# yuanming-hu/exposure

Hardware: AMD Instinct MI355X
Metric: Mpixels/s through 8-step filter chain fwd+bwd (higher is better)
Workload: dtype f16; 1 GPU; 8-step filter chain (E,G,W,S+,T,Ct,BW,C) fwd+bwd, 64x512x512x3 f16 NHWC per GPU, one HIP kernel per filter step and direction; batch_per_gpu=64, global_batch=64, height=512, width=512, parallelism=image-sharded replicas x1 (no data-path collective), weak scaling, launch=hipGraph replay, 10 steps (330 captured launches) per replay, chain_streams=2, transport=none (one process)

## Files before the change

### exposure_amd/csrc/exposure_hip.hip

```cpp
#include <dlfcn.h>
#include <hip/hip_runtime.h>
#include <stdint.h>
#include <stdio.h>
#include <stdlib.h>
#include <string.h>
#include <mutex>
#include <vector>
#include <string>
#include <type_traits>

#include "../../include/exposure_hip.h"
#include "filter_math.h"
#include "pixel_io.h"
#include "kernel_common.h"
#include "host_common.h"

#ifndef EXPO_BWD_MIN_WAVES
#define EXPO_BWD_MIN_WAVES
#endif
#ifndef EXPO_CURVE_BWD_PREFETCH
#define EXPO_CURVE_BWD_PREFETCH 1
#endif
constexpr bool kFwdPrefetch = false;
constexpr bool kBwdPrefetch = true;
constexpr int kAccParts = 4;


namespace expo {

template <class F, typename T, bool VEC, bool PEN, class IO = IoCached>
__device__ __forceinline__ void fwd_body(const T* __restrict__ xi, T* __restrict__ yi,
                                         const float* __restrict__ prm, float* __restrict__ rec,
                                         int hw, int groups) {
  constexpr int PPL = PixTraits<T>::PPL;
  typename F::Prm q;
  if constexpr (!VEC) q = F::load(prm);
  float pen = 0.f;
  const int stride = gridDim.x * kThreads;
  constexpr bool kCurveTab = VEC && F::kLutFloats > 0;
  constexpr int kNC = kCurveTab ? F::NP / kCurveSteps : 1;
  __shared__ float2_lut ftab[kCurveTab ? kWaves : 1][32];
  float2_lut* const tab = ftab[kCurveTab ? (threadIdx.x >> 6) : 0];
  auto compute = [&](float* v, int g) {
    if constexpr (kCurveTab) {
      curve_lut_apply<kNC, PPL>(v, tab);
      if constexpr (PEN) {
#pragma unroll
        for (int j = 0; j < PPL * 3; ++j) {
          const float o = fmaxf(v[j] - 1.0f, 0.0f);
          pen = fmaf(o, o, pen);
        }
      }
      return;
    }
#pragma unroll
    for (int k = 0; k < PPL; ++k) {
      float y[3];
      F::fwd(q, v + 3 * k, y);
#pragma unroll
      for (int c = 0; c < 3; ++c) {
        v[3 * k + c] = y[c];
        if constexpr (PEN) {
          const float o = fmaxf(y[c] - 1.0f, 0.0f);
          pen = fmaf(o, o, pen);
        }
      }
    }
  };
  if constexpr (VEC) {
    const T* const ins[1] = {xi};
    stream_groups<T, 1, true, kFwdPrefetch, IO>(
        ins, yi, hw, blockIdx.x * kThreads + (threadIdx.x & ~63), stride,
        [&](float (&v)[1][PPL * 3], int g) { compute(v[0], g); },
        [&]() {
          q = F::load(prm);
          if constexpr (kCurveTab) curve_lut_build<kNC>(prm[(threadIdx.x & 63) % F::NP], tab);
        });
  } else {
    for (int g = blockIdx.x * kThreads + threadIdx.x; g < groups; g += stride) {
      float v[PPL * 3];
      load_slow<T>(xi, g, hw, v);
      compute(v, g);
      store_slow<T>(yi, g, hw, v);
    }
  }
  if constexpr (PEN) {
    float a[1] = {pen};
    block_reduce_record<1>(a, rec);
  }
}

template <class F, typename T, bool VEC, class IO>
__global__ __launch_bounds__(kThreads) void filter_fwd_kernel(const T* __restrict__ x, T* __restrict__ y,
                                                              const float* __restrict__ params,
                                                              int hw, int groups, int reverse) {
  const int n = reverse ? gridDim.y - 1 - blockIdx.y : blockIdx.y;
  const size_t off = size_t(n) * hw * 3;
  fwd_body<F, T, VEC, false, IO>(x + off, y + off, params + n * F::NP, nullptr, hw, groups);
}

template <class F, typename T, bool VEC, bool HAS_DX, bool PEN, int MODE, class IO = IoCached>
__device__ __forceinline__ void bwd_body(const T* __restrict__ xi, const T* __restrict__ dyi,
                                         T* __restrict__ dxi, const float* __restrict__ prm,
                                         float* __restrict__ rec, int hw, int groups, float pen_scale) {
  constexpr int PPL = PixTraits<T>::PPL;
  const typename F::Prm q = F::load(prm);
  __shared__ __attribute__((aligned(16))) float lut[F::kLutFloats > 0 ? F::kLutFloats : 4];
  constexpr bool kF16X = std::is_same<T, half_t>::value;
// ... 1700 lines not shown
  }
  if (cap != hipStreamCaptureStatusNone) return e;
  probe_helper(e);
  return e;
}
static ForkJoin* fork_join_for_device(hipStream_t caller = nullptr) {
  HelperEntry* e = helper_entry(caller, true);
  return e ? &e->fj : nullptr;
}
static std::mutex g_fork_join_mu;
static int chain_fork(ForkJoin* fj, hipStream_t s) {
  std::lock_guard<std::mutex> lock(g_fork_join_mu);
  HIP_TRY(hipEventRecord(fj->fork, s), "chain fork");
  HIP_TRY(hipStreamWaitEvent(fj->helper, fj->fork, 0), "chain fork");
  return EXPO_OK;
}
static int chain_join(ForkJoin* fj, hipStream_t s) {
  std::lock_guard<std::mutex> lock(g_fork_join_mu);
  HIP_TRY(hipEventRecord(fj->join, fj->helper), "chain join");
  HIP_TRY(hipStreamWaitEvent(s, fj->join, 0), "chain join");
  return EXPO_OK;
}
static bool chain_split(int n, int h, int w, int dtype) {
  static const int forced = getenv("EXPO_CHAIN_STREAMS") ? atoi(getenv("EXPO_CHAIN_STREAMS")) : 0;
  if (n < 2) return false;
  if (forced == 1) return false;
  if (forced >= 2) return true;
  const long bytes = long(n) * h * w * 3L * (dtype == EXPO_F16 ? 2L : 4L);
  return bytes >= (40L << 20) && bytes < (256L << 20);
}

static bool chain_snake(int n, int h, int w, int dtype) {
  static const int forced = getenv("EXPO_CHAIN_SNAKE") ? atoi(getenv("EXPO_CHAIN_SNAKE")) : -1;
  if (forced >= 0) return forced != 0;
  const long bytes = long(n) * h * w * 3L * (dtype == EXPO_F16 ? 2L : 4L);
  return bytes >= (256L << 20);
}

struct ChainChunk { int nb, np, lane; };
struct ChainPlan {
  std::vector<ChainChunk> chunks;
  bool two_lanes = false, snake = false;
};
static ChainPlan chain_plan(int n, int h, int w, int dtype) {
  static const int tile_mib = getenv("EXPO_CHAIN_TILE_MIB") ? atoi(getenv("EXPO_CHAIN_TILE_MIB")) : 96;
  ChainPlan plan;
  const long image_bytes = long(h) * w * 3L * (dtype == EXPO_F16 ? 2L : 4L);
  const long bytes = long(n) * image_bytes;
  int tiles = 1;
  static const long tile_min = long(getenv("EXPO_CHAIN_TILE_MIN_MIB") ? atoi(getenv("EXPO_CHAIN_TILE_MIN_MIB")) : 256) << 20;
  if (tile_mib > 0 && bytes >= tile_min && n > 1) {
    long tile_n = (long(tile_mib) << 20) / image_bytes;
    if (tile_n < 1) tile_n = 1;
    tiles = int((n + tile_n - 1) / tile_n);
  }
  if (tiles == 1) {
    plan.snake = chain_snake(n, h, w, dtype);
    plan.two_lanes = chain_split(n, h, w, dtype);
    const int n0 = plan.two_lanes ? n / 2 : n;
    plan.chunks.push_back({0, n0, 0});
    if (plan.two_lanes) plan.chunks.push_back({n0, n - n0, 1});
    return plan;
  }
  const int base = n / tiles, rem = n % tiles;
  plan.two_lanes = chain_split(base, h, w, dtype);
  int at = 0;
  for (int t = 0; t < tiles; ++t) {
    const int tn = base + (t < rem ? 1 : 0);
    const int n0 = (plan.two_lanes && tn >= 2) ? tn / 2 : tn;
    plan.chunks.push_back({at, n0, 0});
    if (n0 < tn) plan.chunks.push_back({at + n0, tn - n0, 1});
    at += tn;
  }
  return plan;
}

static int chain_fuse_steps(const ChainPlan& plan) {
  static const int forced = env_int("EXPO_CHAIN_FUSE_STEPS", 0);
  if (plan.snake) return 1;
  const int k = forced > 0 ? forced : kChainFuseMax;
  return k < kChainFuseMax ? k : kChainFuseMax;
}

extern "C" {

int expo_version(void) { return EXPO_ABI_VERSION; }

const char* expo_last_error(void) { return g_err.c_str(); }

#ifndef EXPO_SOURCE_DIGEST
#define EXPO_SOURCE_DIGEST "unknown"
#endif
const char* expo_build_info(void) { return EXPO_SOURCE_DIGEST; }

int expo_num_filter_params(int filter_id) {
  if (filter_id < 0 || filter_id >= EXPO_NUM_FILTERS) return -1;
  return kNumParams[filter_id];
}

size_t expo_workspace_bytes(int n, int h, int w, int dtype) {
  if (check_common(n, h, w, dtype) != EXPO_OK || n == 0) return 0;
  const int bx = geom_bx_max(n, h, w, dtype);
  return ws_step_bytes(n, bx);
}

int expo_filter_fwd(int filter_id, const void* x, void* y, const float* params, int n, int h, int w, int dtype,
                    void* stream) {
  if (int rc = check_common(n, h, w, dtype)) return rc;
  if (filter_id < 0 || filter_id >= EXPO_NUM_FILTERS) return fail(EXPO_E_BADARG, "filter_id out of range");
  if (n == 0) return EXPO_OK;
  if (!x || !y || !params) return fail(EXPO_E_BADARG, "null pointer");
  hipStream_t s = static_cast<hipStream_t>(stream);
  return dtype == EXPO_F16 ? fwd_by_id<half_t>(filter_id, x, y, params, n, h, w, s)
                           : fwd_by_id<float>(filter_id, x, y, params, n, h, w, s);
}

static int filter_bwd_common(int filter_id, const void* x, const void* dy, void* dx, const float* params,
                             float* dparams, int n, int h, int w, int dtype, int hsv_grad_mode, void* workspace,
                             size_t workspace_bytes, void* stream, bool accum) {
  if (int rc = check_common(n, h, w, dtype)) return rc;
  if (filter_id < 0 || filter_id >= EXPO_NUM_FILTERS) return fail(EXPO_E_BADARG, "filter_id out of range");
  if (hsv_grad_mode != 0 && hsv_grad_mode != 1) return fail(EXPO_E_BADARG, "hsv_grad_mode must be 0 or 1");
  if (n == 0) return EXPO_OK;
  if (!x || !dy || !params || !dparams) return fail(EXPO_E_BADARG, "null pointer");
  hipStream_t s = static_cast<hipStream_t>(stream);
  const int bx = geom_bx(bwd_geom_kind(filter_id), n, h, w, dtype);
  float* records;
  if (int rc = ws_check(workspace, workspace_bytes, n, bx, 1, &records)) return rc;
  const int rc = dtype == EXPO_F16
                     ? bwd_by_id<half_t>(filter_id, x, dy, dx, params, records, n, h, w, hsv_grad_mode, s)
                     : bwd_by_id<float>(filter_id, x, dy, dx, params, records, n, h, w, hsv_grad_mode, s);
  if (rc) return rc;
  FinishArgs fa{};
  fa.s[0] = FinishStep{params, dparams, nullptr, records, nullptr, kFinFilter, filter_id, accum ? 1 : 0, 0.f, bx};
  return launch_finish(fa, 1, n, s);
}

int expo_filter_bwd(int filter_id, const void* x, const void* dy, void* dx, const float* params, float* dparams,
                    int n, int h, int w, int dtype, int hsv_grad_mode, void* workspace, size_t workspace_bytes,
                    void* stream) {
  return filter_bwd_common(filter_id, x, dy, dx, params, dparams, n, h, w, dtype, hsv_grad_mode, workspace,
                           workspace_bytes, stream, false);
}

int expo_filter_bwd_accumulate(int filter_id, const void* x, const void* dy, void* dx, const float* params,
                               float* dparams, int n, int h, int w, int dtype, int hsv_grad_mode, void* workspace,
                               size_t workspace_bytes, void* stream) {
  return filter_bwd_common(filter_id, x, dy, dx, params, dparams, n, h, w, dtype, hsv_grad_mode, workspace,
                           workspace_bytes, stream, true);
}

int expo_filter_apply_fwd(int filter_id, const void* x, void* y, const float* params, const float* mask_params,
                          float maximum_sharpness, float minimum_strength, int n, int h, int w, int dtype,
                          void* stream) {
  if (int rc = check_common(n, h, w, dtype)) return rc;
  if (filter_id < 0 || filter_id >= EXPO_NUM_FILTERS) return fail(EXPO_E_BADARG, "filter_id out of range");
  if (n == 0) return EXPO_OK;
  if (!x || !y || !params || !mask_params) return fail(EXPO_E_BADARG, "null pointer");
  hipStream_t s = static_cast<hipStream_t>(stream);
  return dtype == EXPO_F16 ? apply_fwd_by_id<half_t>(filter_id, x, y, params, mask_params, maximum_sharpness,
                                                     minimum_strength, n, h, w, s)
                           : apply_fwd_by_id<float>(filter_id, x, y, params, mask_params, maximum_sharpness,
                                                    minimum_strength, n, h, w, s);
}

int expo_filter_apply_bwd(int filter_id, const void* x, const void* dy, void* dx, const float* params,
// ... 159 lines not shown
    int cnt = 1;
    for (int i = 0; i < steps && !rc; i += cnt) {
      cnt = steps - i < fuse ? steps - i : fuse;
      if (cnt > 1) {
        rc = chain_steps_fwd(filter_ids + i, cnt, acts + i, params + i, ck.nb, ck.np, h, w, dtype, n, sp);
      } else {
        const int rev = plan.snake ? (i & 1) : 0;
        const void* xin = static_cast<const char*>(acts[i]) + ioff;
        void* yout = static_cast<char*>(acts[i + 1]) + ioff;
        const float* prm = params[i] + size_t(ck.nb) * kNumParams[filter_ids[i]];
        rc = dtype == EXPO_F16 ? fwd_by_id<half_t>(filter_ids[i], xin, yout, prm, ck.np, h, w, sp, rev, n)
                               : fwd_by_id<float>(filter_ids[i], xin, yout, prm, ck.np, h, w, sp, rev, n);
      }
    }
  }
  if (fj) {
    const int jrc = chain_join(fj, s);
    if (!rc) rc = jrc;
  }
  return rc;
}

int expo_filter_bwd_records(int filter_id, const void* x, const void* dy, void* dx, const float* params, int n,
                            int h, int w, int dtype, int hsv_grad_mode, void* records, size_t records_bytes,
                            void* stream) {
  if (int rc = check_common(n, h, w, dtype)) return rc;
  if (filter_id < 0 || filter_id >= EXPO_NUM_FILTERS) return fail(EXPO_E_BADARG, "filter_id out of range");
  if (hsv_grad_mode != 0 && hsv_grad_mode != 1) return fail(EXPO_E_BADARG, "hsv_grad_mode must be 0 or 1");
  if (n == 0) return EXPO_OK;
  if (!x || !dy || !params) return fail(EXPO_E_BADARG, "null pointer");
  hipStream_t s = static_cast<hipStream_t>(stream);
  const int bx = geom_bx(bwd_geom_kind(filter_id), n, h, w, dtype);
  float* rec;
  if (int rc = ws_check(records, records_bytes, n, bx, 1, &rec)) return rc;
  return dtype == EXPO_F16 ? bwd_by_id<half_t>(filter_id, x, dy, dx, params, rec, n, h, w, hsv_grad_mode, s)
                           : bwd_by_id<float>(filter_id, x, dy, dx, params, rec, n, h, w, hsv_grad_mode, s);
}

int expo_finish_bwd(const int* filter_ids, int steps, const float* const* params, float* const* dparams, int n,
                    int h, int w, int dtype, void* workspace, size_t workspace_bytes, void* stream) {
  if (steps < 0 || !filter_ids || !params || !dparams) return fail(EXPO_E_BADARG, "bad finish arguments");
  if (int rc = check_common(n, h, w, dtype)) return rc;
  if (n == 0 || steps == 0) return EXPO_OK;
  hipStream_t s = static_cast<hipStream_t>(stream);
  const int bx_max = geom_bx_max(n, h, w, dtype);
  float* records;
  if (int rc = ws_check(workspace, workspace_bytes, n, bx_max, steps, &records)) return rc;
  const size_t step_floats = ws_step_bytes(n, bx_max) / sizeof(float);
  for (int i = 0; i < steps; ++i) {
    if (filter_ids[i] < 0 || filter_ids[i] >= EXPO_NUM_FILTERS) return fail(EXPO_E_BADARG, "filter_id out of range");
    if (!params[i] || !dparams[i]) return fail(EXPO_E_BADARG, "null pointer");
  }
  for (int i0 = 0; i0 < steps; i0 += kMaxFinishSteps) {
    const int cnt = steps - i0 < kMaxFinishSteps ? steps - i0 : kMaxFinishSteps;
    FinishArgs fa{};
    for (int k = 0; k < cnt; ++k)
      fa.s[k] = FinishStep{params[i0 + k], dparams[i0 + k], nullptr, records + size_t(i0 + k) * step_floats, nullptr,
                           kFinFilter, filter_ids[i0 + k], 0, 0.f,
                           geom_bx(bwd_geom_kind(filter_ids[i0 + k]), n, h, w, dtype)};
    if (int rc = launch_finish(fa, cnt, n, s)) return rc;
  }
  return EXPO_OK;
}

int expo_chain_bwd(const int* filter_ids, int steps, void* const* acts, void* const* grads,
                   const float* const* params, float* const* dparams, int n, int h, int w, int dtype,
                   int hsv_grad_mode, void* workspace, size_t workspace_bytes, void* stream) {
  if (steps < 0 || !filter_ids || !acts || !grads || !params || !dparams)
    return fail(EXPO_E_BADARG, "bad chain arguments");
  if (int rc = check_common(n, h, w, dtype)) return rc;
  if (hsv_grad_mode != 0 && hsv_grad_mode != 1) return fail(EXPO_E_BADARG, "hsv_grad_mode must be 0 or 1");
  if (n == 0 || steps == 0) return EXPO_OK;
  hipStream_t s = static_cast<hipStream_t>(stream);
  for (int i = 0; i < steps; ++i) {
    if (filter_ids[i] < 0 || filter_ids[i] >= EXPO_NUM_FILTERS) return fail(EXPO_E_BADARG, "filter_id out of range");
    if (!dparams[i] || !acts[i] || !grads[i + 1] || !params[i]) return fail(EXPO_E_BADARG, "null pointer");
  }
  const int bx_max = geom_bx_max(n, h, w, dtype);
  float* records;
  if (int rc = ws_check(workspace, workspace_bytes, n, bx_max, steps, &records)) return rc;
  const size_t step_floats = ws_step_bytes(n, bx_max) / sizeof(float);
  const size_t esz = dtype == EXPO_F16 ? 2 : 4;
  const ChainPlan plan = chain_plan(n, h, w, dtype);
  ForkJoin* fj = plan.two_lanes ? fork_join_for_device(s) : nullptr;
  if (plan.two_lanes && !fj) return fail(EXPO_E_HIP, "helper stream unavailable");
  if (fj) {
    if (int rc = chain_fork(fj, s)) return rc;
  }
  int rc = EXPO_OK;
  for (size_t c = 0; c < plan.chunks.size() && !rc; ++c) {
    const ChainChunk& ck = plan.chunks[c];
    hipStream_t sp = ck.lane ? fj->helper : s;
    const size_t ioff = size_t(ck.nb) * h * w * 3 * esz;
    for (int i = steps - 1; i >= 0 && !rc; --i) {
      const int rev = plan.snake ? ((i + 1) & 1) : 0;
      const int bx = geom_bx(bwd_geom_kind(filter_ids[i]), n, h, w, dtype);
      float* rec = records + size_t(i) * step_floats + size_t(ck.nb) * bx * kWsSlots;
      const void* xin = static_cast<const char*>(acts[i]) + ioff;
      const void* gin = static_cast<const char*>(grads[i + 1]) + ioff;
      void* gout = grads[i] ? static_cast<char*>(grads[i]) + ioff : nullptr;
      const float* prm = params[i] + size_t(ck.nb) * kNumParams[filter_ids[i]];
      rc = dtype == EXPO_F16
               ? bwd_by_id<half_t>(filter_ids[i], xin, gin, gout, prm, rec, ck.np, h, w, hsv_grad_mode, sp, rev, n)
               : bwd_by_id<float>(filter_ids[i], xin, gin, gout, prm, rec, ck.np, h, w, hsv_grad_mode, sp, rev, n);
    }
  }
  if (fj) {
    const int jrc = chain_join(fj, s);
    if (!rc) rc = jrc;
  }
  if (rc) return rc;
  return expo_finish_bwd(filter_ids, steps, params, dparams, n, h, w, dtype, workspace, workspace_bytes, stream);
}

int expo_critic_stats(const void* x, float* stats, int n, int h, int w, int dtype, void* workspace,
                      size_t workspace_bytes, void* stream) {
  if (int rc = check_common(n, h, w, dtype)) return rc;
  if (n == 0) return EXPO_OK;
  if (!x || !stats) return fail(EXPO_E_BADARG, "null pointer");
  hipStream_t s = static_cast<hipStream_t>(stream);
  return dtype == EXPO_F16 ? stats_t<half_t>(x, stats, n, h, w, workspace, workspace_bytes, s)
                           : stats_t<float>(x, stats, n, h, w, workspace, workspace_bytes, s);
}

int expo_overexposure_penalty(const void* y, float* penalty, int n, int h, int w, int dtype, void* workspace,
                              size_t workspace_bytes, void* stream) {
  if (int rc = check_common(n, h, w, dtype)) return rc;
  if (n == 0) return EXPO_OK;
  if (!y || !penalty) return fail(EXPO_E_BADARG, "null pointer");
  hipStream_t s = static_cast<hipStream_t>(stream);
  return dtype == EXPO_F16 ? penalty_t<half_t>(y, penalty, n, h, w, workspace, workspace_bytes, s)
                           : penalty_t<float>(y, penalty, n, h, w, workspace, workspace_bytes, s);
}

int expo_vignet_apply_fwd(const void* x, void* y, const float* mask_params, float maximum_sharpness, int masking, int n,
                          int h, int w, int dtype, void* stream) {
  if (int rc = check_common(n, h, w, dtype)) return rc;
  if (n == 0) return EXPO_OK;
  if (!x || !y || !mask_params) return fail(EXPO_E_BADARG, "null pointer");
  hipStream_t s = static_cast<hipStream_t>(stream);
  return dtype == EXPO_F16 ? vignet_fwd_t<half_t>(x, y, mask_params, maximum_sharpness, masking, n, h, w, s)
                           : vignet_fwd_t<float>(x, y, mask_params, maximum_sharpness, masking, n, h, w, s);
}

int expo_vignet_apply_bwd(const void* x, const void* dy, void* dx, const float* mask_params, float* dmask_params,
                          float maximum_sharpness, int masking, int n, int h, int w, int dtype, void* workspace,
                          size_t workspace_bytes, void* stream) {
  if (int rc = check_common(n, h, w, dtype)) return rc;
  if (n == 0) return EXPO_OK;
  if (!x || !dy || !mask_params || !dmask_params) return fail(EXPO_E_BADARG, "null pointer");
  hipStream_t s = static_cast<hipStream_t>(stream);
  return dtype == EXPO_F16 ? vignet_bwd_t<half_t>(x, dy, dx, mask_params, dmask_params, maximum_sharpness, masking, n, h,
                                                  w, workspace, workspace_bytes, s)
                           : vignet_bwd_t<float>(x, dy, dx, mask_params, dmask_params, maximum_sharpness, masking, n, h,
                                                 w, workspace, workspace_bytes, s);
}

int expo_overexposure_penalty_bwd(const void* y, const float* dpenalty, void* dy, int n, int h, int w, int dtype,
                                  void* stream) {
  if (int rc = check_common(n, h, w, dtype)) return rc;
  if (n == 0) return EXPO_OK;
  if (!y || !dpenalty || !dy) return fail(EXPO_E_BADARG, "null pointer");
  hipStream_t s = static_cast<hipStream_t>(stream);
  return dtype == EXPO_F16 ? penalty_bwd_t<half_t>(y, dpenalty, dy, n, h, w, s)
                           : penalty_bwd_t<float>(y, dpenalty, dy, n, h, w, s);
}

int expo_critic_stats_bwd(const void* x, const float* stats, const float* dstats, void* dx, int n, int h, int w,
                          int dtype, void* stream) {
  if (int rc = check_common(n, h, w, dtype)) return rc;
  if (n == 0) return EXPO_OK;
  if (!x || !stats || !dstats || !dx) return fail(EXPO_E_BADARG, "null pointer");
  hipStream_t s = static_cast<hipStream_t>(stream);
  return dtype == EXPO_F16 ? stats_bwd_t<half_t>(x, stats, dstats, dx, n, h, w, s)
                           : stats_bwd_t<float>(x, stats, dstats, dx, n, h, w, s);
}

// ... 67 lines not shown
```

### exposure_amd/csrc/host_common.h

```cpp
#pragma once
#include <hip/hip_runtime.h>
#include <stdint.h>
#include <stdlib.h>

#include <initializer_list>
#include <string>

#include "../../include/exposure_hip.h"
#include "kernel_common.h"

namespace expo {

extern thread_local std::string g_err;

inline int fail(int code, const char* what) {
  g_err = what;
  return code;
}
inline int fail_hip(hipError_t e, const char* where) {
  g_err = std::string(where) + ": " + hipGetErrorString(e);
  return EXPO_E_HIP;
}
#define HIP_TRY(expr, where)                         \
  do {                                               \
    hipError_t e_ = (expr);                          \
    if (e_ != hipSuccess) return fail_hip(e_, where); \
  } while (0)

constexpr int kNumParams[EXPO_NUM_FILTERS] = {1, 1, 3, 1, 8, 1, 1, 24, 2};

struct Geom {
  int hw, groups, blocks_x;
  bool vec;
  bool stream;
};

inline int env_int(const char* name, int dflt) {
  const char* v = getenv(name);
  if (!v || !*v) return dflt;
  const int x = atoi(v);
  return x > 0 ? x : dflt;
}

inline long stream_min_bytes() {
  static const long v = env_int("EXPO_STREAM_MIN_BYTES", 8 << 20);
  return v;
}

constexpr int kMaxReduceBlocksX = 1024;
enum GeomKind {
  kGeomMap = 0,
  kGeomReduce = 1,
  kGeomReadReduce = 2,
  kGeomDispatch = 3,
  kGeomReduceTone = 4,
  kGeomReduceColor = 5,
  kGeomApply = 6,
  kGeomFusedBwd = 7,
  kNumGeomKinds = 8
};
inline int bwd_geom_kind(int filter_id) { return filter_id == 4 ? kGeomReduceTone : filter_id == 7 ? kGeomReduceColor : kGeomReduce; }

template <typename T>
inline Geom make_geom(int n, int h, int w, std::initializer_list<const void*> ptrs, int kind) {
  const bool reduces = kind != kGeomMap;
  constexpr int PPL = PixTraits<T>::PPL;
  Geom g;
  g.hw = h * w;
  g.groups = (g.hw + PPL - 1) / PPL;
  g.vec = (g.hw % VecTraits<T>::PPV) == 0;
  for (const void* p : ptrs) g.vec = g.vec && (p == nullptr || (reinterpret_cast<uintptr_t>(p) & 3) == 0);
  const int max_bx = (g.groups + kThreads - 1) / kThreads;
  static const int gpt_kind[kNumGeomKinds] = {
      env_int("EXPO_FWD_GROUPS_PER_THREAD", 1),       env_int("EXPO_BWD_GROUPS_PER_THREAD", 1),
      env_int("EXPO_RED_GROUPS_PER_THREAD", 4),       env_int("EXPO_DISPATCH_GROUPS_PER_THREAD", 4),
      env_int("EXPO_TONE_GROUPS_PER_THREAD", 2),      env_int("EXPO_COLOR_GROUPS_PER_THREAD", 2),
      env_int("EXPO_APPLY_GROUPS_PER_THREAD", 4),     env_int("EXPO_FUSED_BWD_GROUPS_PER_THREAD", 8)};
  int gpt = gpt_kind[kind >= 0 && kind < kNumGeomKinds ? kind : kGeomReduce];
  static const bool bwd_gpt_forced = getenv("EXPO_BWD_GROUPS_PER_THREAD") != nullptr;
  if (kind == kGeomReduce && !bwd_gpt_forced && long(n) * g.hw * 3L * long(sizeof(T)) >= (256L << 20) && gpt < 4) gpt = 4;
  int bx = (g.groups + kThreads * gpt - 1) / (kThreads * gpt);
  const long want = 1024;
  if (long(bx) * n < want) bx = int((want + n - 1) / n);
  if (bx > max_bx) bx = max_bx;
  if (reduces && bx > kMaxReduceBlocksX) bx = kMaxReduceBlocksX;
  if (bx < 1) bx = 1;
  g.blocks_x = bx;
  g.stream = g.vec && long(n) * g.hw * 3L * long(sizeof(T)) >= stream_min_bytes();
  return g;
}

int chain_records(void* workspace, size_t workspace_bytes, int n, int h, int w, int dtype, int steps, float** records,
                  size_t* step_floats);
int finish_chain_fused(const int32_t* ids, const float* params, float* dparams, const float* records,
                       size_t step_floats, int steps, int n, int blocks_x, hipStream_t s);

constexpr int kChainFuseMax = 8;
bool chain_steps_vec_path(void* const* acts, int steps, int h, int w, int dtype);
int chain_steps_fwd(const int* ids, int cnt, void* const* acts, const float* const* params, int nb, int np, int h,
                    int w, int dtype, int n_geom, hipStream_t s);

inline int check_common(int n, int h, int w, int dtype) {
  if (n < 0 || h < 1 || w < 1) return fail(EXPO_E_BADARG, "n >= 0, h >= 1, w >= 1 required");
  if (n > 65535) return fail(EXPO_E_BADARG, "n > 65535 not supported (grid.y)");
  if (dtype != EXPO_F16 && dtype != EXPO_F32) return fail(EXPO_E_BADDTYPE, "dtype must be EXPO_F16 or EXPO_F32");
  const long image_bytes = long(h) * long(w) * 3L * (dtype == EXPO_F16 ? 2L : 4L);
  if (image_bytes > (1L << 31) - 8192) return fail(EXPO_E_BADARG, "one image must be smaller than 2 GiB");
  return EXPO_OK;
}

}
```

### exposure_amd/csrc/kernel_common.h

```cpp
#pragma once
#include <hip/hip_runtime.h>
#include <stdint.h>

#include "filter_math.h"
#include "pixel_io.h"

namespace expo {

constexpr int kThreads = 256;
constexpr int kWaves = kThreads / 64;

template <int N, int M>
__device__ __forceinline__ void reduce_scatter_step(float* acc, int lane) {
  constexpr int H = (N + 1) / 2;
  const bool upper = (lane & M) != 0;
#pragma unroll
  for (int j = 0; j < H; ++j) {
    const float lo = acc[j];
    const float hi = (j + H < N) ? acc[j + H] : 0.0f;
    const float keep = upper ? hi : lo;
    const float send = upper ? lo : hi;
    acc[j] = keep + __shfl_xor(send, M, 64);
  }
}
__host__ __device__ constexpr int reduce_scatter_index(int N, int lane) {
  const int n1 = (N + 1) / 2, n2 = (n1 + 1) / 2, n3 = (n2 + 1) / 2, n4 = (n3 + 1) / 2, n5 = (n4 + 1) / 2;
  int l = 0;
  bool ok = true;
  if (n4 > 1) { l += (lane & 2) ? n5 : 0; ok = ok && l < n4; }
  if (n3 > 1) { l += (lane & 4) ? n4 : 0; ok = ok && l < n3; }
  if (n2 > 1) { l += (lane & 8) ? n3 : 0; ok = ok && l < n2; }
  if (n1 > 1) { l += (lane & 16) ? n2 : 0; ok = ok && l < n1; }
  if (N > 1) { l += (lane & 32) ? n1 : 0; ok = ok && l < N; }
  return ok ? l : -1;
}
constexpr bool reduce_scatter_map_is_complete(int N) {
  for (int a = 0; a < N; ++a) {
    bool held = false;
    for (int lane = 0; lane < 64; lane += 2) held = held || reduce_scatter_index(N, lane) == a;
    if (!held) return false;
  }
  for (int lane = 0; lane < 64; ++lane)
    if (reduce_scatter_index(N, lane) >= N) return false;
  return true;
}
static_assert(reduce_scatter_map_is_complete(1) && reduce_scatter_map_is_complete(2) && reduce_scatter_map_is_complete(3) &&
              reduce_scatter_map_is_complete(5) && reduce_scatter_map_is_complete(6) && reduce_scatter_map_is_complete(7) &&
              reduce_scatter_map_is_complete(8) && reduce_scatter_map_is_complete(9) && reduce_scatter_map_is_complete(14) &&
              reduce_scatter_map_is_complete(24) && reduce_scatter_map_is_complete(30) && reduce_scatter_map_is_complete(32),
              "wave_reduce_scatter: slot map");

template <int N>
__device__ __forceinline__ int wave_reduce_scatter(float* acc, int lane) {
  constexpr int n1 = (N + 1) / 2, n2 = (n1 + 1) / 2, n3 = (n2 + 1) / 2, n4 = (n3 + 1) / 2, n5 = (n4 + 1) / 2;
  static_assert(n5 == 1, "at most 32 accumulators");
  if constexpr (N > 1) reduce_scatter_step<N, 32>(acc, lane); else acc[0] += __shfl_xor(acc[0], 32, 64);
  if constexpr (n1 > 1) reduce_scatter_step<n1, 16>(acc, lane); else acc[0] += __shfl_xor(acc[0], 16, 64);
  if constexpr (n2 > 1) reduce_scatter_step<n2, 8>(acc, lane); else acc[0] += __shfl_xor(acc[0], 8, 64);
  if constexpr (n3 > 1) reduce_scatter_step<n3, 4>(acc, lane); else acc[0] += __shfl_xor(acc[0], 4, 64);
  if constexpr (n4 > 1) reduce_scatter_step<n4, 2>(acc, lane); else acc[0] += __shfl_xor(acc[0], 2, 64);
  acc[0] += __shfl_xor(acc[0], 1, 64);
  int l = 0;
  bool ok = true;
  if constexpr (n4 > 1) { l += (lane & 2) ? n5 : 0; ok = ok && l < n4; }
  if constexpr (n3 > 1) { l += (lane & 4) ? n4 : 0; ok = ok && l < n3; }
  if constexpr (n2 > 1) { l += (lane & 8) ? n3 : 0; ok = ok && l < n2; }
  if constexpr (n1 > 1) { l += (lane & 16) ? n2 : 0; ok = ok && l < n1; }
  if constexpr (N > 1) { l += (lane & 32) ? n1 : 0; ok = ok && l < N; }
  return ok ? l : -1;
}

constexpr int kWsSlots = 32;

template <int NACC>
__device__ __forceinline__ void block_reduce_record(float* acc, float* __restrict__ records_img) {
  static_assert(NACC <= kWsSlots, "one record per block");
  __shared__ float red[kWaves][NACC];
  const int lane = threadIdx.x & 63, wv = threadIdx.x >> 6;
  const int idx = wave_reduce_scatter<NACC>(acc, lane);
  if ((lane & 1) == 0 && idx >= 0) red[wv][idx] = acc[0];
  __syncthreads();
  if (threadIdx.x < NACC) {
    float v = 0.f;
#pragma unroll
    for (int k = 0; k < kWaves; ++k) v += red[k][threadIdx.x];
    records_img[size_t(blockIdx.x) * kWsSlots + threadIdx.x] = v;
  }
}

template <int NC>
__device__ __forceinline__ void curve_lut_build(float klane, float2_lut* tab) {
  constexpr int L = kCurveSteps;
  const int lane = threadIdx.x & 63;
// ... 85 lines not shown
```

Baseline: 33260 Mpixels/s.

## Fuse consecutive element-wise backward filter steps into one kernel

Adds a chain_steps_bwd kernel that runs up to four consecutive element-wise backward steps (gamma, white balance, tf1-mode saturation) in one pass. The upstream gradient is kept in registers between steps instead of being written and re-read, and each step's parameter-gradient partials are reduced to its own record slot. Host planning groups fusable runs, checks for aliasing between gradient and activation buffers, and skips redundant gradient stores. This removes launches and intermediate gradient traffic, at the cost of more registers and loads of several activation tensors per iteration.

```diff
diff --git a/exposure_amd/csrc/chain_steps_bwd.hip b/exposure_amd/csrc/chain_steps_bwd.hip
--- /dev/null
+++ b/exposure_amd/csrc/chain_steps_bwd.hip
@@ -0,0 +1,213 @@
+#include <hip/hip_runtime.h>
+#include <stdint.h>
+
+#include "../../include/exposure_hip.h"
+#include "filter_math.h"
+#include "pixel_io.h"
+#include "kernel_common.h"
+#include "host_common.h"
+
+namespace expo {
+
+struct ChainStepsBwdArgs {
+  const void* dy;
+  const void* x[kChainBwdFuseMax];
+  void* dx[kChainBwdFuseMax];
+  const float* prm[kChainBwdFuseMax];
+  float* rec[kChainBwdFuseMax];
+  int id[kChainBwdFuseMax];
+  int steps, hw;
+};
+
+template <typename T>
+constexpr int chain_bwd_parts() { return kAccParts < PixTraits<T>::PPL ? kAccParts : PixTraits<T>::PPL; }
+
+constexpr int kChainBwdPrmFloats = 3;
+template <class F>
+struct ChainBwdPrmRaw { float f[sizeof(typename F::Prm) / sizeof(float)]; };
+template <class F>
+__device__ __forceinline__ void chain_bwd_load_prm(const float* __restrict__ prm, float (&out)[kChainBwdPrmFloats]) {
+  static_assert(sizeof(typename F::Prm) <= sizeof(out) && sizeof(typename F::Prm) % sizeof(float) == 0, "Prm is floats");
+  const ChainBwdPrmRaw<F> r = __builtin_bit_cast(ChainBwdPrmRaw<F>, F::load(prm));
+#pragma unroll
+  for (int j = 0; j < int(sizeof(r.f) / sizeof(float)); ++j) out[j] = r.f[j];
+}
+
+template <class F, typename T, int MODE, int NA>
+__device__ __forceinline__ void chain_bwd_step(const float (&pq)[kChainBwdPrmFloats], const RawGroup& xr, RawGroup& g,
+                                               float (&acc)[chain_bwd_parts<T>()][NA]) {
+  static_assert(F::NACC <= NA && !F::kHasGroupBwd && F::kLutFloats == 0, "element-wise filters only");
+  constexpr int PPL = PixTraits<T>::PPL, kParts = chain_bwd_parts<T>();
+  ChainBwdPrmRaw<F> raw;
+#pragma unroll
+  for (int j = 0; j < int(sizeof(raw.f) / sizeof(float)); ++j) raw.f[j] = pq[j];
+  const typename F::Prm q = __builtin_bit_cast(typename F::Prm, raw);
+  float v[PPL * 3], d[PPL * 3];
+  unpack<T>(xr, v);
+  unpack<T>(g, d);
+#pragma unroll
+  for (int k = 0; k < PPL; ++k) {
+    float dx[3];
+    F::bwd(q, nullptr, v + 3 * k, d + 3 * k, dx, acc[k % kParts], MODE);
+#pragma unroll
+    for (int c = 0; c < 3; ++c) d[3 * k + c] = dx[c];
+  }
+  g = pack<T>(d);
+}
+
+template <int NACC, typename T, int NA>
+__device__ __forceinline__ void chain_bwd_reduce(float (&acc)[chain_bwd_parts<T>()][NA], float* __restrict__ rec) {
+  constexpr int kParts = chain_bwd_parts<T>();
+#pragma unroll
+  for (int p = 1; p < kParts; ++p)
+#pragma unroll
+    for (int j = 0; j < NACC; ++j) acc[0][j] += acc[p][j];
+  block_reduce_record<NACC>(acc[0], rec);
+}
+
+template <typename T, class IO, int NA, bool PF>
+__global__ __launch_bounds__(kThreads) void chain_steps_bwd_kernel(const ChainStepsBwdArgs a) {
+  constexpr int PPL = PixTraits<T>::PPL, kParts = chain_bwd_parts<T>(), kMax = kChainBwdFuseMax;
+  const int n = blockIdx.y;
+  const int hw = a.hw;
+  const size_t off = size_t(n) * hw * 3;
+  const int lane = threadIdx.x & 63;
+  const int image_bytes = hw * 3 * int(sizeof(T));
+#if EXPO_FP16_OVFL
+  if constexpr (sizeof(T) == 2) __builtin_amdgcn_s_setreg(1 | (23 << 6) | (0 << 11), 1);
+#endif
+  float acc[kMax][kParts][NA];
+#pragma unroll
+  for (int s = 0; s < kMax; ++s)
+#pragma unroll
+    for (int p = 0; p < kParts; ++p)
+#pragma unroll
+      for (int j = 0; j < NA; ++j) acc[s][p][j] = 0.f;
+
+  float pq[kMax][kChainBwdPrmFloats];
+#pragma unroll
+  for (int s = 0; s < kMax; ++s) {
+#pragma unroll
+    for (int j = 0; j < kChainBwdPrmFloats; ++j) pq[s][j] = 0.f;
+    if (s < a.steps) {
+      switch (a.id[s]) {
+        case 1: chain_bwd_load_prm<GammaF>(a.prm[s] + n * GammaF::NP, pq[s]); break;
+        case 2: chain_bwd_load_prm<WhiteBalanceF>(a.prm[s] + n * WhiteBalanceF::NP, pq[s]); break;
+        case 3: chain_bwd_load_prm<SatPlusF>(a.prm[s] + n * SatPlusF::NP, pq[s]); break;
+        default: break;
+      }
+    }
+  }
+  const __amdgpu_buffer_rsrc_t rdy = make_image_rsrc(static_cast<const T*>(a.dy) + off, hw);
+  const __amdgpu_buffer_rsrc_t rx0 = make_image_rsrc(static_cast<const T*>(a.x[0]) + off, hw);
+  const int stride = gridDim.x * kThreads;
+  int gw = blockIdx.x * kThreads + (threadIdx.x & ~63);
+  if (gw * PPL < hw) {
+    RawGroup cg = load_raw<IO::kLoadDy>(rdy, chunk_byte_offset<T>(gw, lane));
+    RawGroup cx0 = load_raw<IO::kLoadX>(rx0, chunk_byte_offset<T>(gw, lane));
+    while (true) {
+      const int boff = chunk_byte_offset<T>(gw, lane);
+      RawGroup xs[kMax];
+      xs[0] = cx0;
+#pragma unroll
+      for (int s = 1; s < kMax; ++s)
+        if (s < a.steps) xs[s] = load_raw<IO::kLoadX>(make_image_rsrc(static_cast<const T*>(a.x[s]) + off, hw), boff);
+      const int gn = gw + stride;
+      const bool more = gn * PPL < hw;
+      RawGroup ng = cg, nx0 = cx0;
+      const bool partial = (gw + 64) * PPL > hw;
+      RawGroup g = cg;
+#pragma unroll
+      for (int s = 0; s < kMax; ++s) {
+        if (s < a.steps) {
+          if (PF && s == 0 && more) {
+            ng = load_raw<IO::kLoadDy>(rdy, chunk_byte_offset<T>(gn, lane));
+            nx0 = load_raw<IO::kLoadX>(rx0, chunk_byte_offset<T>(gn, lane));
+          }
+#define EXPO_CASE(ID, F, MODE) \
+  case ID: chain_bwd_step<F, T, MODE, NA>(pq[s], xs[s], g, acc[s]); break;
+          switch (a.id[s]) {
+            EXPO_CASE(1, GammaF, 0)
+            case 2:
+              if constexpr (NA >= 3) chain_bwd_step<WhiteBalanceF, T, 0, NA>(pq[s], xs[s], g, acc[s]);
+              break;
+            EXPO_CASE(3, SatPlusF, 0)
+            default: break;
+          }
+#undef EXPO_CASE
+          if (partial) {
+#pragma unroll
+            for (int j = 0; j < 4; ++j)
+              if (boff + j * 768 >= image_bytes) g.q[j] = u32x3_t{0u, 0u, 0u};
+          }
+          if (a.dx[s]) store_raw<IO::kStore>(make_image_rsrc(static_cast<T*>(a.dx[s]) + off, hw), boff, g);
+        }
+      }
+      if (!more) break;
+      if (!PF) {
+        ng = load_raw<IO::kLoadDy>(rdy, chunk_byte_offset<T>(gn, lane));
+        nx0 = load_raw<IO::kLoadX>(rx0, chunk_byte_offset<T>(gn, lane));
+      }
+      gw = gn;
+      cg = ng;
+      cx0 = nx0;
+    }
+  }
+#pragma unroll
+  for (int s = 0; s < kMax; ++s) {
+    if (s < a.steps) {
+      if (s > 0) __syncthreads();
+      float* const rec = a.rec[s] + size_t(n) * gridDim.x * kWsSlots;
+      switch (a.id[s]) {
+        case 2:
+          if constexpr (NA >= 3) chain_bwd_reduce<3, T, NA>(acc[s], rec);
+          break;
+        default: chain_bwd_reduce<1, T, NA>(acc[s], rec); break;
+      }
+    }
+  }
+}
+
+template <typename T>
+static int chain_steps_bwd_t(const ChainStepsBwdArgs& a, bool wide, int np, int h, int w, int n_geom, hipStream_t s) {
+  const Geom g = make_geom<T>(n_geom, h, w, {}, kGeomReduce);
+  const dim3 grid(g.blocks_x, np), block(kThreads);
+  const bool pf = kBwdPrefetch && g.stream && long(g.blocks_x) * kThreads < g.groups;
+#define EXPO_L(IO, PF)                                                                          \
+  do {                                                                                          \
+    if (wide) hipLaunchKernelGGL((chain_steps_bwd_kernel<T, IO, 3, PF>), grid, block, 0, s, a); \
+    else hipLaunchKernelGGL((chain_steps_bwd_kernel<T, IO, 1, PF>), grid, block, 0, s, a);      \
+  } while (0)
+  if (pf) EXPO_L(IoStream, true);
+  else if (g.stream) EXPO_L(IoStream, false);
+  else EXPO_L(IoCached, false);
+#undef EXPO_L
+  HIP_TRY(hipGetLastError(), "chain_steps_bwd launch");
+  return EXPO_OK;
+}
+
+int chain_steps_bwd(const int* ids, int cnt, void* const* acts, void* const* grads, const float* const* params,
+                    float* const* recs, const bool* store, int nb, int np, int h, int w, int dtype, int hsv_grad_mode,
+                    int n_geom, hipStream_t s) {
+  if (cnt < 1 || cnt > kChainBwdFuseMax) return fail(EXPO_E_BADARG, "chain_steps_bwd: step count");
+  const size_t ioff = size_t(nb) * h * w * 3 * (dtype == EXPO_F16 ? 2 : 4);
+  ChainStepsBwdArgs a{};
+  bool wide = false;
+  a.dy = static_cast<const char*>(grads[cnt]) + ioff;
+  for (int k = 0; k < cnt; ++k) {
+    const int i = cnt - 1 - k;
+    if (!chain_bwd_fusable(ids[i], hsv_grad_mode)) return fail(EXPO_E_BADARG, "chain_steps_bwd: filter not served");
+    a.x[k] = static_cast<const char*>(acts[i]) + ioff;
+    a.dx[k] = (grads[i] && store[i]) ? static_cast<char*>(grads[i]) + ioff : nullptr;
+    a.prm[k] = params[i] + size_t(nb) * kNumParams[ids[i]];
+    a.rec[k] = recs[i];
+    a.id[k] = ids[i];
+    wide = wide || kNumParams[ids[i]] > 1;
+  }
+  a.steps = cnt;
+  a.hw = h * w;
+  return dtype == EXPO_F16 ? chain_steps_bwd_t<half_t>(a, wide, np, h, w, n_geom, s)
+                           : chain_steps_bwd_t<float>(a, wide, np, h, w, n_geom, s);
+}
+
+}
diff --git a/exposure_amd/csrc/exposure_hip.hip b/exposure_amd/csrc/exposure_hip.hip
--- a/exposure_amd/csrc/exposure_hip.hip
+++ b/exposure_amd/csrc/exposure_hip.hip
@@ -22,8 +22,6 @@
 #define EXPO_CURVE_BWD_PREFETCH 1
 #endif
 constexpr bool kFwdPrefetch = false;
-constexpr bool kBwdPrefetch = true;
-constexpr int kAccParts = 4;
 
 
 namespace expo {
@@ -1890,6 +1888,46 @@
   return k < kChainFuseMax ? k : kChainFuseMax;
 }
 
+static int chain_fuse_bwd_steps(const ChainPlan& plan) {
+  static const int forced = env_int("EXPO_CHAIN_FUSE_BWD_STEPS", 0);
+  if (plan.snake) return 1;
+  const int k = forced > 0 ? forced : kChainBwdFuseMax;
+  return k < kChainBwdFuseMax ? k : kChainBwdFuseMax;
+}
+
+struct BwdRun { int first, cnt; };
+static int chain_bwd_runs(const int* ids, int steps, int mode, void* const* acts, void* const* grads,
+                          size_t tensor_bytes, int cap, BwdRun* runs, char* store) {
+  int count = 0;
+  for (int i = 0; i < steps; ++i) store[i] = 1;
+  auto overlap = [tensor_bytes](const void* a, const void* b) {
+    const uintptr_t pa = reinterpret_cast<uintptr_t>(a), pb = reinterpret_cast<uintptr_t>(b);
+    return pa < pb + tensor_bytes && pb < pa + tensor_bytes;
+  };
+  for (int last = steps - 1; last >= 0;) {
+    int first = last;
+    if (cap > 1 && chain_bwd_fusable(ids[last], mode))
+      while (first > 0 && last - first + 1 < cap && chain_bwd_fusable(ids[first - 1], mode)) --first;
+    bool ok = true;
+    for (int i = first; i <= last && ok && first < last; ++i) {
+      if (!grads[i]) continue;
+      for (int j = first; j <= last && ok; ++j) ok = !overlap(grads[i], acts[j]);
+      for (int j = first; j <= last + 1 && ok; ++j)
+        ok = !grads[j] || grads[j] == grads[i] || !overlap(grads[i], grads[j]);
+    }
+    if (!ok) {
+      for (int i = last; i >= first; --i) runs[count++] = {i, 1};
+    } else {
+      runs[count++] = {first, last - first + 1};
+      for (int i = first + 1; i <= last; ++i)
+        for (int j = first; j < i; ++j)
+          if (grads[j] && grads[j] == grads[i]) store[i] = 0;
+    }
+    last = first - 1;
+  }
+  return count;
+}
+
 extern "C" {
 
 int expo_version(void) { return EXPO_ABI_VERSION; }
@@ -2215,17 +2253,48 @@
   const size_t step_floats = ws_step_bytes(n, bx_max) / sizeof(float);
   const size_t esz = dtype == EXPO_F16 ? 2 : 4;
   const ChainPlan plan = chain_plan(n, h, w, dtype);
+  bool vec = chain_steps_vec_path(acts, steps, h, w, dtype);
+  for (int i = 0; i <= steps && vec; ++i) vec = (reinterpret_cast<uintptr_t>(grads[i]) & 3) == 0;
+  constexpr int kInlineSteps = 32;
+  BwdRun runs_inline[kInlineSteps];
+  char store_inline[kInlineSteps];
+  std::vector<BwdRun> runs_long;
+  std::vector<char> store_long;
+  BwdRun* runs = runs_inline;
+  char* store = store_inline;
+  if (steps > kInlineSteps) {
+    runs_long.resize(size_t(steps));
+    store_long.resize(size_t(steps));
+    runs = runs_long.data();
+    store = store_long.data();
+  }
+  const int cap = vec ? chain_fuse_bwd_steps(plan) : 1;
+  const int nruns =
+      chain_bwd_runs(filter_ids, steps, hsv_grad_mode, acts, grads, size_t(n) * h * w * 3 * esz, cap, runs, store);
   ForkJoin* fj = plan.two_lanes ? fork_join_for_device(s) : nullptr;
   if (plan.two_lanes && !fj) return fail(EXPO_E_HIP, "helper stream unavailable");
   if (fj) {
     if (int rc = chain_fork(fj, s)) return rc;
   }
   int rc = EXPO_OK;
+  const int bx_reduce = geom_bx(kGeomReduce, n, h, w, dtype);
   for (size_t c = 0; c < plan.chunks.size() && !rc; ++c) {
     const ChainChunk& ck = plan.chunks[c];
     hipStream_t sp = ck.lane ? fj->helper : s;
     const size_t ioff = size_t(ck.nb) * h * w * 3 * esz;
-    for (int i = steps - 1; i >= 0 && !rc; --i) {
+    for (int r = 0; r < nruns && !rc; ++r) {
+      const int i = runs[r].first;
+      if (runs[r].cnt > 1) {
+        float* recs[kChainBwdFuseMax];
+        bool st[kChainBwdFuseMax];
+        for (int k = 0; k < runs[r].cnt; ++k) {
+          recs[k] = records + size_t(i + k) * step_floats + size_t(ck.nb) * bx_reduce * kWsSlots;
+          st[k] = store[i + k] != 0;
+        }
+        rc = chain_steps_bwd(filter_ids + i, runs[r].cnt, acts + i, grads + i, params + i, recs, st, ck.nb, ck.np, h, w,
+                             dtype, hsv_grad_mode, n, sp);
+        continue;
+      }
       const int rev = plan.snake ? ((i + 1) & 1) : 0;
       const int bx = geom_bx(bwd_geom_kind(filter_ids[i]), n, h, w, dtype);
       float* rec = records + size_t(i) * step_floats + size_t(ck.nb) * bx * kWsSlots;
diff --git a/exposure_amd/csrc/host_common.h b/exposure_amd/csrc/host_common.h
--- a/exposure_amd/csrc/host_common.h
+++ b/exposure_amd/csrc/host_common.h
@@ -100,6 +100,15 @@
 int chain_steps_fwd(const int* ids, int cnt, void* const* acts, const float* const* params, int nb, int np, int h,
                     int w, int dtype, int n_geom, hipStream_t s);
 
+inline bool chain_bwd_fusable(int filter_id, int hsv_grad_mode) {
+  return filter_id == EXPO_FILTER_GAMMA || filter_id == EXPO_FILTER_WB ||
+         (filter_id == EXPO_FILTER_SATPLUS && hsv_grad_mode == EXPO_HSV_GRAD_TF1);
+}
+constexpr int kChainBwdFuseMax = 4;
+int chain_steps_bwd(const int* ids, int cnt, void* const* acts, void* const* grads, const float* const* params,
+                    float* const* recs, const bool* store, int nb, int np, int h, int w, int dtype, int hsv_grad_mode,
+                    int n_geom, hipStream_t s);
+
 inline int check_common(int n, int h, int w, int dtype) {
   if (n < 0 || h < 1 || w < 1) return fail(EXPO_E_BADARG, "n >= 0, h >= 1, w >= 1 required");
   if (n > 65535) return fail(EXPO_E_BADARG, "n > 65535 not supported (grid.y)");
diff --git a/exposure_amd/csrc/kernel_common.h b/exposure_amd/csrc/kernel_common.h
--- a/exposure_amd/csrc/kernel_common.h
+++ b/exposure_amd/csrc/kernel_common.h
@@ -9,6 +9,9 @@
 
 constexpr int kThreads = 256;
 constexpr int kWaves = kThreads / 64;
+
+constexpr bool kBwdPrefetch = true;
+constexpr int kAccParts = 4;
 
 template <int N, int M>
 __device__ __forceinline__ void reduce_scatter_step(float* acc, int lane) {
```

Result: faster. 34760 Mpixels/s, median of 6 (+4.5%).

## Fuse consecutive elementwise backward steps into one multi-step kernel

Applied to the files above, without the earlier changes.

Adds a kernel that runs up to four consecutive backward steps (gamma, white balance, saturation) in one pass, keeping the gradient in registers between steps. The host planner groups fusable runs, checks buffers for aliasing, and skips intermediate gradient stores that later steps overwrite. This removes kernel launches and the re-reading of intermediate gradients from memory. In exchange, register pressure rises and the planner adds host-side logic; the path is disabled in snake mode and for unaligned buffers.

```diff
diff --git a/exposure_amd/csrc/chain_steps_bwd.hip b/exposure_amd/csrc/chain_steps_bwd.hip
--- /dev/null
+++ b/exposure_amd/csrc/chain_steps_bwd.hip
@@ -0,0 +1,195 @@
+#include <hip/hip_runtime.h>
+#include <stdint.h>
+
+#include "../../include/exposure_hip.h"
+#include "filter_math.h"
+#include "pixel_io.h"
+#include "kernel_common.h"
+#include "host_common.h"
+
+namespace expo {
+
+constexpr int kChainBwdAccMax = 3;
+static_assert(GammaF::NACC == 1 && SatPlusF::NACC == 1 && WhiteBalanceF::NACC == kChainBwdAccMax && GammaF::NP == 1 &&
+                  SatPlusF::NP == 1 && WhiteBalanceF::NP == 3,
+              "a step slot holds three accumulators and three parameters");
+
+struct ChainStepsBwdArgs {
+  const void* dy;
+  const void* x[kChainBwdFuseMax];
+  void* dx[kChainBwdFuseMax];
+  const float* prm[kChainBwdFuseMax];
+  float* rec[kChainBwdFuseMax];
+  int id[kChainBwdFuseMax];
+  int steps, hw;
+};
+
+__device__ __forceinline__ void opaque(RawGroup& r) {
+#pragma unroll
+  for (int j = 0; j < 4; ++j) asm("" : "+v"(r.q[j]));
+}
+
+template <typename T, class IO, int STEPS>
+__global__ __launch_bounds__(kThreads) void chain_steps_bwd_kernel(const ChainStepsBwdArgs a) {
+  constexpr int PPL = PixTraits<T>::PPL, PPV = VecTraits<T>::PPV;
+  constexpr int kParts = kAccParts < PPL ? kAccParts : PPL;
+  static_assert(STEPS >= 2 && STEPS <= kChainBwdFuseMax, "a run holds 2 to kChainBwdFuseMax steps");
+  constexpr int kMax = STEPS;
+  const int n = blockIdx.y;
+  const int hw = a.hw;
+  const size_t off = size_t(n) * hw * 3;
+  const int lane = threadIdx.x & 63;
+#if EXPO_FP16_OVFL
+  if constexpr (sizeof(T) == 2) __builtin_amdgcn_s_setreg(1 | (23 << 6) | (0 << 11), 1);
+#endif
+  float acc[kMax][kParts][kChainBwdAccMax];
+#pragma unroll
+  for (int st = 0; st < kMax; ++st)
+#pragma unroll
+    for (int p = 0; p < kParts; ++p)
+#pragma unroll
+      for (int j = 0; j < kChainBwdAccMax; ++j) acc[st][p][j] = 0.f;
+
+  const int stride = gridDim.x * kThreads;
+  int gw = blockIdx.x * kThreads + (threadIdx.x & ~63);
+  bool work = gw * PPL < hw;
+  const __amdgpu_buffer_rsrc_t rdy = make_image_rsrc(static_cast<const T*>(a.dy) + off, hw);
+  RawGroup xs{}, g{};
+  if (work) {
+    const int boff = chunk_byte_offset<T>(gw, lane);
+    xs = load_raw<IO::kLoadX>(make_image_rsrc(static_cast<const T*>(a.x[0]) + off, hw), boff);
+    g = load_raw<IO::kLoadDy>(rdy, boff);
+  }
+  float pr[kMax][3];
+#pragma unroll
+  for (int st = 0; st < kMax; ++st) {
+    pr[st][0] = pr[st][1] = pr[st][2] = 0.f;
+    const int np = a.id[st] == 2 ? WhiteBalanceF::NP : 1;
+    const float* const p = a.prm[st] + size_t(n) * np;
+    pr[st][0] = p[0];
+    if (np > 1) pr[st][1] = p[1];
+    if (np > 2) pr[st][2] = p[2];
+  }
+
+  while (work) {
+    const int boff = chunk_byte_offset<T>(gw, lane);
+    const int gn = gw + stride;
+    const bool more = gn * PPL < hw;
+    const bool partial = (gw + 64) * PPL > hw;
+    RawGroup gnext{};
+#pragma unroll
+    for (int st = 0; st < kMax; ++st) {
+      const bool last = st + 1 == kMax;
+      RawGroup xn{};
+      if (!last) {
+        xn = load_raw<IO::kLoadX>(make_image_rsrc(static_cast<const T*>(a.x[st + 1 < kMax ? st + 1 : 0]) + off, hw), boff);
+      } else if (more) {
+        const int bn = chunk_byte_offset<T>(gn, lane);
+        xn = load_raw<IO::kLoadX>(make_image_rsrc(static_cast<const T*>(a.x[0]) + off, hw), bn);
+        gnext = load_raw<IO::kLoadDy>(rdy, bn);
+      }
+      T* const dxp = static_cast<T*>(a.dx[st]);
+      float v[PPL * 3], d[PPL * 3];
+#define EXPO_CASE(ID, F)                                                                          \
+  case ID: {                                                                                      \
+    const typename F::Prm q = F::load(pr[st]);                                                    \
+    opaque(xs);                                                                                   \
+    opaque(g);                                                                                    \
+    unpack<T>(xs, v);                                                                             \
+    unpack<T>(g, d);                                                                              \
+    _Pragma("unroll") for (int k = 0; k < PPL; ++k) {                                             \
+      float dx[3];                                                                                \
+      F::bwd(q, nullptr, v + 3 * k, d + 3 * k, dx, acc[st][k % kParts], 0);                       \
+      _Pragma("unroll") for (int c = 0; c < 3; ++c) d[3 * k + c] = dx[c];                         \
+    }                                                                                             \
+    g = pack<T>(d);                                                                               \
+    opaque(g);                                                                                    \
+  } break;
+      switch (a.id[st]) {
+        EXPO_CASE(1, GammaF)
+        EXPO_CASE(2, WhiteBalanceF)
+        EXPO_CASE(3, SatPlusF)
+        default: break;
+      }
+#undef EXPO_CASE
+      if (partial) {
+#pragma unroll
+        for (int j = 0; j < 4; ++j)
+          if (!live_pixel<T, true>(gw + lane, j * PPV, lane, hw)) g.q[j] = u32x3_t{0u, 0u, 0u};
+      }
+      if (dxp != nullptr) store_raw<IO::kStore>(make_image_rsrc(dxp + off, hw), boff, g);
+      xs = xn;
+    }
+    if (!more) break;
+    g = gnext;
+    gw = gn;
+  }
+
+#pragma unroll
+  for (int st = 0; st < kMax; ++st) {
+    if (st > 0) __syncthreads();
+#pragma unroll
+    for (int p = 1; p < kParts; ++p)
+#pragma unroll
+      for (int j = 0; j < kChainBwdAccMax; ++j) acc[st][0][j] += acc[st][p][j];
+    float* const rec = a.rec[st] + size_t(n) * gridDim.x * kWsSlots;
+    switch (a.id[st]) {
+      case 2: block_reduce_record<WhiteBalanceF::NACC>(acc[st][0], rec); break;
+      default: block_reduce_record<1>(acc[st][0], rec); break;
+    }
+  }
+}
+
+template <typename T>
+static int chain_steps_bwd_t(const ChainStepsBwdArgs& a, int np, int h, int w, int n_geom, hipStream_t s) {
+  const Geom g = make_geom<T>(n_geom, h, w, {}, kGeomReduce);
+  const dim3 grid(g.blocks_x, np), block(kThreads);
+#define EXPO_L(STEPS)                                                                                  \
+  do {                                                                                                 \
+    if (g.stream) hipLaunchKernelGGL((chain_steps_bwd_kernel<T, IoStream, STEPS>), grid, block, 0, s, a); \
+    else hipLaunchKernelGGL((chain_steps_bwd_kernel<T, IoCached, STEPS>), grid, block, 0, s, a);       \
+  } while (0)
+  static_assert(kChainBwdFuseMax == 4, "one instantiation per run length");
+  switch (a.steps) {
+    case 2: EXPO_L(2); break;
+    case 3: EXPO_L(3); break;
+    default: EXPO_L(4); break;
+  }
+#undef EXPO_L
+  HIP_TRY(hipGetLastError(), "chain_steps_bwd launch");
+  return EXPO_OK;
+}
+
+bool chain_steps_bwd_vec_path(void* const* acts, void* const* grads, int steps, int h, int w, int dtype) {
+  const int ppv = dtype == EXPO_F16 ? VecTraits<half_t>::PPV : VecTraits<float>::PPV;
+  if ((long(h) * w) % ppv != 0) return false;
+  for (int k = 0; k < steps; ++k)
+    if ((reinterpret_cast<uintptr_t>(acts[k]) & 3) != 0) return false;
+  for (int k = 0; k <= steps; ++k)
+    if ((reinterpret_cast<uintptr_t>(grads[k]) & 3) != 0) return false;
+  return true;
+}
+
+int chain_steps_bwd(const int* ids, int cnt, void* const* acts, void* const* grads, const uint8_t* store,
+                    const float* const* params, float* const* recs, int nb, int np, int h, int w, int dtype, int mode,
+                    int n_geom, hipStream_t s) {
+  if (cnt < 2 || cnt > kChainBwdFuseMax) return fail(EXPO_E_BADARG, "chain_steps_bwd: step count");
+  const size_t ioff = size_t(nb) * h * w * 3 * (dtype == EXPO_F16 ? 2 : 4);
+  ChainStepsBwdArgs a{};
+  a.dy = static_cast<const char*>(grads[cnt]) + ioff;
+  for (int k = 0; k < cnt; ++k) {
+    const int i = cnt - 1 - k;
+    if (!chain_bwd_fusable(ids[i], mode)) return fail(EXPO_E_BADARG, "chain_steps_bwd: filter id");
+    a.x[k] = static_cast<const char*>(acts[i]) + ioff;
+    a.dx[k] = (store[i] && grads[i]) ? static_cast<char*>(grads[i]) + ioff : nullptr;
+    a.prm[k] = params[i] + size_t(nb) * kNumParams[ids[i]];
+    a.rec[k] = recs[i];
+    a.id[k] = ids[i];
+  }
+  a.steps = cnt;
+  a.hw = h * w;
+  return dtype == EXPO_F16 ? chain_steps_bwd_t<half_t>(a, np, h, w, n_geom, s)
+                           : chain_steps_bwd_t<float>(a, np, h, w, n_geom, s);
+}
+
+}
diff --git a/exposure_amd/csrc/exposure_hip.hip b/exposure_amd/csrc/exposure_hip.hip
--- a/exposure_amd/csrc/exposure_hip.hip
+++ b/exposure_amd/csrc/exposure_hip.hip
@@ -23,7 +23,6 @@
 #endif
 constexpr bool kFwdPrefetch = false;
 constexpr bool kBwdPrefetch = true;
-constexpr int kAccParts = 4;
 
 
 namespace expo {
@@ -1890,6 +1889,13 @@
   return k < kChainFuseMax ? k : kChainFuseMax;
 }
 
+static int chain_bwd_fuse_steps(const ChainPlan& plan) {
+  static const int forced = env_int("EXPO_CHAIN_FUSE_BWD_STEPS", 0);
+  if (plan.snake) return 1;
+  const int k = forced > 0 ? forced : kChainBwdFuseMax;
+  return k < kChainBwdFuseMax ? k : kChainBwdFuseMax;
+}
+
 extern "C" {
 
 int expo_version(void) { return EXPO_ABI_VERSION; }
@@ -2215,6 +2221,32 @@
   const size_t step_floats = ws_step_bytes(n, bx_max) / sizeof(float);
   const size_t esz = dtype == EXPO_F16 ? 2 : 4;
   const ChainPlan plan = chain_plan(n, h, w, dtype);
+  const int fuse = chain_steps_bwd_vec_path(acts, grads, steps, h, w, dtype) ? chain_bwd_fuse_steps(plan) : 1;
+  const size_t tensor_bytes = size_t(n) * h * w * 3 * esz;
+  auto touch = [tensor_bytes](const void* p, const void* q) {
+    if (!p || !q) return false;
+    const uintptr_t a = reinterpret_cast<uintptr_t>(p), b = reinterpret_cast<uintptr_t>(q);
+    return (a < b ? b - a : a - b) < tensor_bytes;
+  };
+  auto clash = [&touch](const void* p, const void* q) { return p != q && touch(p, q); };
+  std::vector<int> run(steps, 1);
+  std::vector<uint8_t> store(steps, 1);
+  for (int i = steps - 1; i >= 0; i -= run[i]) {
+    if (fuse < 2 || !chain_bwd_fusable(filter_ids[i], hsv_grad_mode)) continue;
+    int cnt = 1;
+    while (cnt < fuse && i - cnt >= 0 && chain_bwd_fusable(filter_ids[i - cnt], hsv_grad_mode)) {
+      const int cand = i - cnt;
+      bool ok = !clash(grads[cand], grads[i + 1]) && !touch(grads[cand], acts[cand]);
+      for (int k = i; k > cand && ok; --k)
+        ok = !clash(grads[cand], grads[k]) && !touch(grads[cand], acts[k]) && !touch(grads[k], acts[cand]);
+      if (!ok) break;
+      ++cnt;
+    }
+    run[i] = cnt;
+    for (int k = i; k > i - cnt + 1; --k)
+      for (int j = 0; j < k && store[k]; ++j)
+        if (grads[j] == grads[k]) store[k] = 0;
+  }
   ForkJoin* fj = plan.two_lanes ? fork_join_for_device(s) : nullptr;
   if (plan.two_lanes && !fj) return fail(EXPO_E_HIP, "helper stream unavailable");
   if (fj) {
@@ -2225,7 +2257,16 @@
     const ChainChunk& ck = plan.chunks[c];
     hipStream_t sp = ck.lane ? fj->helper : s;
     const size_t ioff = size_t(ck.nb) * h * w * 3 * esz;
-    for (int i = steps - 1; i >= 0 && !rc; --i) {
+    for (int i = steps - 1; i >= 0 && !rc; i -= run[i]) {
+      if (run[i] > 1) {
+        const int cnt = run[i], lo = i - cnt + 1;
+        const int bx = geom_bx(kGeomReduce, n, h, w, dtype);
+        float* recs[kChainBwdFuseMax];
+        for (int k = 0; k < cnt; ++k) recs[k] = records + size_t(lo + k) * step_floats + size_t(ck.nb) * bx * kWsSlots;
+        rc = chain_steps_bwd(filter_ids + lo, cnt, acts + lo, grads + lo, store.data() + lo, params + lo, recs, ck.nb,
+                             ck.np, h, w, dtype, hsv_grad_mode, n, sp);
+        continue;
+      }
       const int rev = plan.snake ? ((i + 1) & 1) : 0;
       const int bx = geom_bx(bwd_geom_kind(filter_ids[i]), n, h, w, dtype);
       float* rec = records + size_t(i) * step_floats + size_t(ck.nb) * bx * kWsSlots;
diff --git a/exposure_amd/csrc/host_common.h b/exposure_amd/csrc/host_common.h
--- a/exposure_amd/csrc/host_common.h
+++ b/exposure_amd/csrc/host_common.h
@@ -100,6 +100,15 @@
 int chain_steps_fwd(const int* ids, int cnt, void* const* acts, const float* const* params, int nb, int np, int h,
                     int w, int dtype, int n_geom, hipStream_t s);
 
+inline bool chain_bwd_fusable(int filter_id, int hsv_grad_mode) {
+  return filter_id == 1 || filter_id == 2 || (filter_id == 3 && hsv_grad_mode == 0);
+}
+constexpr int kChainBwdFuseMax = 4;
+bool chain_steps_bwd_vec_path(void* const* acts, void* const* grads, int steps, int h, int w, int dtype);
+int chain_steps_bwd(const int* ids, int cnt, void* const* acts, void* const* grads, const uint8_t* store,
+                    const float* const* params, float* const* recs, int nb, int np, int h, int w, int dtype, int mode,
+                    int n_geom, hipStream_t s);
+
 inline int check_common(int n, int h, int w, int dtype) {
   if (n < 0 || h < 1 || w < 1) return fail(EXPO_E_BADARG, "n >= 0, h >= 1, w >= 1 required");
   if (n > 65535) return fail(EXPO_E_BADARG, "n > 65535 not supported (grid.y)");
diff --git a/exposure_amd/csrc/kernel_common.h b/exposure_amd/csrc/kernel_common.h
--- a/exposure_amd/csrc/kernel_common.h
+++ b/exposure_amd/csrc/kernel_common.h
@@ -9,6 +9,7 @@
 
 constexpr int kThreads = 256;
 constexpr int kWaves = kThreads / 64;
+constexpr int kAccParts = 4;
 
 template <int N, int M>
 __device__ __forceinline__ void reduce_scatter_step(float* acc, int lane) {
```

After: 31820 Mpixels/s before, 33450 Mpixels/s after (median of 6 runs). +5.1%, better.
